# noahares/raxtax

Measured on AMD Instinct MI355X. Metric: classified queries/sec (whole node), higher is better.
Workload: dtype u32 bit-planes + f64

## Files before the change

### include/raxtax_hip.h

```cpp
#ifndef RAXTAX_HIP_H
#define RAXTAX_HIP_H

#include <stddef.h>
#include <stdint.h>

#ifdef __cplusplus
extern "C" {
#endif

#define RTX_ABI_VERSION 6
#define RTX_NUM_KMERS 65536u
#define RTX_MAX_DEPTH 32u

#define RTX_OK 0
#define RTX_ERR_INVALID (-1)
#define RTX_ERR_HIP (-2)
#define RTX_ERR_NO_DEVICE (-3)
#define RTX_ERR_OOM (-4)
#define RTX_ERR_PARSE (-5)
#define RTX_ERR_DEPTH (-6)
#define RTX_ERR_STATE (-7)
#define RTX_ERR_TOO_LONG (-8)
#define RTX_ERR_SENDER (-9)
#define RTX_RETRY_CHUNK 1
// ... 89 lines not shown
#define RTX_OPT_TILE_SKIP 10
#define RTX_OPT_LOCATOR 12
#define RTX_OPT_TILE_PRUNE 13
#define RTX_OPT_FINE_BOUNDS 17
#define RTX_OPT_RECORDS 18
#define RTX_OPT_OVERLAP 19
#define RTX_OPT_MIN_SUB_BATCHES 20
#define RTX_OPT_TWO_LEVEL_BOUNDS 21
#define RTX_OPT_PRUNE_SELF_SAMPLE 22
#define RTX_OPT_RUN_AHEAD 23
#define RTX_OPT_DEVICE_TEXT 24
#define RTX_OPT_STRAND 25
#define RTX_OPT_NEAREST 26
#define RTX_NO_REF 0xFFFFFFFFu
#define RTX_OPT_DEREP 27
int rtx_index_set_option(rtx_index *index, int option, uint64_t value);

int rtx_index_self_sample(rtx_index *index, const uint8_t *seq_bytes, const uint64_t *seq_off, uint64_t n_refs, uint32_t n_sample, double *live_fraction);
int rtx_index_prune_verdict(const rtx_index *index, int *pruning, double *live_fraction);
int rtx_index_run_ahead_stats(const rtx_index *index, uint64_t *enqueued_ahead, uint64_t *abandoned);
#define RTX_DEFAULT_SEGMENT_CLASSES 1
#define RTX_DEFAULT_EXACT_HASH_MASK 2
#define RTX_DEFAULT_DEREP_HASH_MASK 3
int rtx_set_default_option(int option, uint64_t value);

typedef struct {
    uint32_t n_queries;
    uint64_t n_rows;
    const uint32_t *t;
    const uint8_t *status;
// ... 164 lines not shown
```

### raxtax_amd/_lib.py

```python
from __future__ import annotations

import ctypes as C
from pathlib import Path

import numpy as np

PKG = Path(__file__).resolve().parent
import os as _os

LIB_PATH = Path(_os.environ.get("RTX_LIB_PATH") or PKG / "libraxtax_hip.so")

RTX_MAX_DEPTH = 32
RTX_NUM_KMERS = 65536
RTX_OK = 0
RTX_ERR_INVALID, RTX_ERR_HIP, RTX_ERR_NO_DEVICE, RTX_ERR_OOM = -1, -2, -3, -4
RTX_ERR_PARSE, RTX_ERR_DEPTH, RTX_ERR_STATE, RTX_ERR_TOO_LONG = -5, -6, -7, -8
RTX_SKIP_EXACT_MATCHES = 1
RTX_RAW_CONFIDENCE = 2
RTX_TEXT_TSV = 4
RTX_Q_OK, RTX_Q_NO_KMERS, RTX_Q_ALL_KMERS = 0, 1, 2
RTX_OPT_DEREP = 27
RTX_DEFAULT_DEREP_HASH_MASK = 3
STAGES = ("kmer_extract", "hit_count", "prob_table", "taxon_prefix", "lineage_walk", "tile_bounds", "tile_prune", "exact_match", "order", "pair_union")

u8p = C.POINTER(C.c_uint8)
u16p = C.POINTER(C.c_uint16)
u32p = C.POINTER(C.c_uint32)
u64p = C.POINTER(C.c_uint64)
f64p = C.POINTER(C.c_double)
f32p = C.POINTER(C.c_float)


class NodesView(C.Structure):
    _fields_ = [("n_nodes", C.c_uint32), ("node_begin", u32p), ("node_end", u32p), ("node_first_child", u32p),
                ("node_n_children", u32p), ("node_parent", u32p), ("node_type", u8p)]

# ... 180 lines not shown
```

### raxtax_amd/api.py

```python
from __future__ import annotations

import ctypes as C
from dataclasses import dataclass
from typing import Callable, List, Optional, Sequence, Tuple

import numpy as np

from . import _lib
from ._lib import (RTX_MAX_DEPTH, RTX_RAW_CONFIDENCE, RTX_SKIP_EXACT_MATCHES, NodesView, ResultView, RtxError, check,
                   f32p, f64p, ptr, u8p, u16p, u32p, u64p)


def _flatten(seqs: Sequence[np.ndarray]) -> Tuple[np.ndarray, np.ndarray]:
    off = np.zeros(len(seqs) + 1, dtype=np.uint64)
    if len(seqs):
        off[1:] = np.cumsum([len(s) for s in seqs], dtype=np.uint64)
    flat = np.zeros(max(int(off[-1]), 1), dtype=np.uint8)
    for i, s in enumerate(seqs):
        flat[int(off[i]):int(off[i + 1])] = np.asarray(s, dtype=np.uint8)
    return flat, off


class Tree:

# ... 210 lines not shown

DEFAULT_SEGMENT_CLASSES = 1


class Index:

    nearest_on = False

    def __init__(self, tree: Tree, device: int = 0, sub_batch: int = 0, prob_mode: int = 0,
                 stage_timing: bool = False, cluster: Optional[bool] = None, segment_classes=None,
                 packed_counts: Optional[bool] = None,
                 tile_skip: Optional[bool] = None, hit_pair=None, locator: Optional[bool] = None, tile_prune: Optional[bool] = None,
                 debug_taps: bool = False, device_exact: Optional[bool] = None, fine_bounds: Optional[bool] = None,
                 records: Optional[int] = None, overlap: Optional[bool] = None, two_level: Optional[int] = None,
                 prune_self_sample: Optional[bool] = None, device_text: bool = False, strand: str = "plus",
                 nearest: bool = False, derep: bool = False):
        self._lib = _lib.load()
        self.tree = tree
        if segment_classes is None:
            segment_classes = DEFAULT_SEGMENT_CLASSES
        check(self._lib.rtx_set_default_option(1, int(segment_classes)))
        h = C.c_void_p()
        check(self._lib.rtx_index_create_from_tree(device, tree._h, C.byref(h)))
        self._h = h
        self.n_refs = self._lib.rtx_index_num_refs(self._h)
        if sub_batch:
            check(self._lib.rtx_index_set_batch(self._h, sub_batch))
        if prob_mode:
            check(self._lib.rtx_index_set_option(self._h, 2, prob_mode))
        if stage_timing:
            check(self._lib.rtx_index_set_option(self._h, 6, 1))
# ... 25 lines not shown
            check(self._lib.rtx_index_set_option(self._h, 19, int(overlap)))
        if two_level is not None:
            check(self._lib.rtx_index_set_option(self._h, 21, int(two_level)))
        if prune_self_sample is not None:
            check(self._lib.rtx_index_set_option(self._h, 22, int(prune_self_sample)))
        if strand not in ("plus", "both"):
            raise ValueError(f"strand must be 'plus' or 'both', not {strand!r}")
        self.strand = strand
        if strand == "both":
            check(self._lib.rtx_index_set_option(self._h, 25, 1))
        self.nearest_on = bool(nearest)
        if nearest:
            check(self._lib.rtx_index_set_option(self._h, 26, 1))
        if derep:
            check(self._lib.rtx_index_set_option(self._h, _lib.RTX_OPT_DEREP, 1))
        self._view = ResultView()
        self._keep = None

    @property
    def prune_verdict(self):
        on, frac = C.c_int(), C.c_double()
        check(self._lib.rtx_index_prune_verdict(self._h, C.byref(on), C.byref(frac)))
        return bool(on.value), float(frac.value)

    @property
    def run_ahead_stats(self):
        a, b = C.c_uint64(), C.c_uint64()
        check(self._lib.rtx_index_run_ahead_stats(self._h, C.byref(a), C.byref(b)))
        return int(a.value), int(b.value)

# ... 402 lines not shown
```

### raxtax_amd/csrc/rtx_api_batch.hip

```cpp
#include "rtx_index.hpp"

#ifndef RTX_B2_HEAVY_PER_ATILE
#define RTX_B2_HEAVY_PER_ATILE 4u
#endif

namespace rtxi {

int bind(rtx_index *ix) {
    if (!ix) { set_error("null index handle"); return RTX_ERR_INVALID; }
    RTX_HIP(hipSetDevice(ix->device));
    return RTX_OK;
}

int ensure_events(rtx_index *ix, size_t count) {
    while (ix->events.size() < count) {
        hipEvent_t e;
        RTX_HIP(hipEventCreate(&e));
        ix->events.push_back(e);
    }
    return RTX_OK;
}


SubBatch sub_batch_of(rtx_index *ix, uint32_t sb, bool timed) {
// ... 70 lines not shown
    kp.rstride = k.rstride;
    kp.dmask = sc.d_dmask.p;
    kp.srows = sc.d_srows.p;
    kp.nsparse = sc.d_nsparse.p;
    kp.t = sc.d_t.p;
    kp.nrows = sc.d_nrows.p;
    kp.hq = r.d_hq.p;
    kp.t_all = r.d_t_all.p;
    kp.nrows_all = r.d_nrows_all.p;
    kp.hist = sc.d_hist.p;
    kp.hstride = k.hstride;
    return kp;
}

static bool run_prunes(const rtx_index *ix, const rtx_index::BatchClass &k) { return k.prune && !ix->dbg_full_run; }
static bool on_records_path(const rtx_index *ix, const rtx_index::BatchClass &k, const rtx_index::Scratch &sc) { return run_prunes(ix, k) && k.rec && sc.d_rec.p != nullptr; }
static bool on_diet(const rtx_index *ix, const rtx_index::BatchClass &k, const rtx_index::Scratch &sc) { return on_records_path(ix, k, sc) && k.diet && sc.d_cnt_row.p != nullptr; }

static RecordRef record_ref(const rtx_index *ix, const rtx_index::Scratch &sc, const rtx_index::ResultSet &r) { return RecordRef{sc.d_rec_nslots.p, sc.d_rec_slots.p, sc.d_rec_cnt.p, sc.d_rec.p, ix->rec_slots(), ix->rec_seg_len, r.d_flags.p}; }
static ProbTables prob_tables(const rtx_index *ix) { return ProbTables{ix->d_tab_cmf.p, ix->d_tab_ratio.p, ix->d_tab_off.p, ix->d_tab_moff.p, ix->d_tab_ilo.p, ix->d_tab_sat.p, ix->tab_tmax}; }

int enqueue_kmer(rtx_index *ix, const SubBatch &b, hipStream_t s) {
    KmerParams kp = kmer_params(ix, b);
    kp.mode = run_prunes(ix, *b.cls) && ix->seg_blocks ? 1u : 0u;
    if (b.timed_all) RTX_HIP(hipEventRecord(stage_event(ix, b, RTX_STAGE_KMER_EXTRACT, 0), s));
    launch_kmer_extract(s, kp, b.nq);
    if (b.timed_all) RTX_HIP(hipEventRecord(stage_event(ix, b, RTX_STAGE_KMER_EXTRACT, 1), s));
    return RTX_OK;
}

static HitParams hit_params(rtx_index *ix, const SubBatch &b, uint32_t flags) {
    rtx_index::Scratch &sc = ix->sc[b.set];
    rtx_index::ResultSet &r = ix->res();
    const rtx_index::BatchClass &k = *b.cls;
    HitParams hp{};
    hp.bitmap = ix->d_bitmap.p;
    hp.stride_bytes = ix->stride_bytes;
    hp.n_rows1 = ix->n_rows + 1;
    hp.n_refs = ix->n_refs;
    hp.ref_base = ix->ref_lo;
    hp.rows = sc.d_rows.p;
// ... 132 lines not shown
    fp.live_words = LiveLayout{ix->ntiles}.words();
    fp.prune_thr = sc.d_prune_thr.p;
    fp.fine_n_refs = ix->n_refs;
    fp.fine_ref_ntiles = ix->ntiles;
    fp.fine_stats = ix->d_prune_stats.p + 2 * kPruneStatCopies * 8;
    return fp;
}

int enqueue_hit(rtx_index *ix, const SubBatch &b, uint32_t flags, hipStream_t s, int part, hipStream_t s_mid) {
    rtx_index::Scratch &sc = ix->sc[b.set];
    rtx_index::ResultSet &r = ix->res();
    const rtx_index::BatchClass &k = *b.cls;
    ix->last_set = b.set;
    HitParams hp = hit_params(ix, b, flags);
    const bool prune = run_prunes(ix, k);
    if (k.pair && part != 2) {
        if (b.timed_all) RTX_HIP(hipEventRecord(stage_event(ix, b, RTX_STAGE_PAIR_UNION, 0), s));
        launch_pair_union(s, sc.d_rows.p, sc.d_nrows.p, k.rstride, b.nq, sc.d_urec.p, sc.d_nu.p, 2u * k.rstride);
        if (b.timed_all) RTX_HIP(hipEventRecord(stage_event(ix, b, RTX_STAGE_PAIR_UNION, 1), s));
    }
    if (b.timed && !prune) RTX_HIP(hipEventRecord(stage_event(ix, b, RTX_STAGE_HIT_COUNT, 0), s));
    if (part != 0 && !prune) { set_error("internal: a split run without tile pruning"); return RTX_ERR_STATE; }
    if (prune) {
        if (part != 2) {
            const HitParams up = bounds_params(ix, sc, hp);
            if (b.timed) RTX_HIP(hipEventRecord(stage_event(ix, b, RTX_STAGE_TILE_BOUNDS, 0), s));
            ix->two_level_used = part == 0 && ix->two_level_opt && ix->d_abitmap.p && ix->d_bbitmap.p && ix->n_refs == ix->n_total && k.planes <= kBounds2MaxPlanes;
            if (ix->two_level_used) {
                const bool heavy_ok = sc.d_heavy.p && sc.d_heavy_items.p && sc.d_heavy_items.n >= HeavyItemsLayout(b.nq, ix->u_ntiles).total();
                launch_bounds2(s, bounds2_params(ix, sc, up, heavy_ok), b.nq, k.planes, up, ix->u_ntiles, heavy_ok ? sc.d_heavy_items.p : nullptr);
            } else {
// ... 1003 lines not shown
```

### raxtax_amd/csrc/rtx_api_debug.hip

```cpp
#include "rtx_index.hpp"

extern "C" {

int rtx_batch_stage_times(rtx_index *ix, float ms[RTX_NUM_STAGES], uint32_t launches[RTX_NUM_STAGES]) {
    int rc = bind(ix);
    if (rc) return rc;
    if (!ix->synced) { set_error("rtx_batch_stage_times: batch not synchronised"); return RTX_ERR_STATE; }
    for (int s = 0; s < RTX_NUM_STAGES; s++) { ms[s] = 0.f; launches[s] = 0; }
    for (uint32_t sb = 0; sb < ix->n_sub_last; sb++) {
        const rtx_index::BatchClass &kc = ix->cls[ix->plan[sb].cls];
        for (int s = 0; s < RTX_NUM_STAGES; s++) {
            if (s == RTX_STAGE_EXACT_MATCH) {
                if (sb != 0 || !ix->dev_exact_used || !ix->stage_timing) continue;
            } else if (s == RTX_STAGE_ORDER) {
                if (sb != 0 || !ix->stage_timing) continue;
            } else if (s == RTX_STAGE_PAIR_UNION) {
                if (!kc.pair || !ix->stage_timing) continue;
            } else if (s == RTX_STAGE_TILE_BOUNDS || s == RTX_STAGE_TILE_PRUNE ? !kc.prune : (s != RTX_STAGE_HIT_COUNT && !ix->stage_timing)) continue;
            float t = 0.f;
            RTX_HIP(hipEventElapsedTime(&t, ix->events[((size_t)sb * RTX_NUM_STAGES + s) * 2],
                                        ix->events[((size_t)sb * RTX_NUM_STAGES + s) * 2 + 1]));
            ms[s] += t;
            launches[s]++;
        }
    }
    return RTX_OK;
}

int rtx_batch_nearest_time(rtx_index *ix, float *ms, uint32_t *launches) {
    if (!ix || !ms || !launches) { set_error("null argument"); return RTX_ERR_INVALID; }
    int rc = bind(ix);
    if (rc) return rc;
// ... 139 lines not shown
        if (row == 0xFFFFFFFFu) { set_error("debug tap: the query holds no row of the counts buffer (records path)"); return RTX_ERR_STATE; }
        slot = row;
    }
    if (!ix->packs(k.planes)) { *out = sc.d_counts.p + (size_t)slot * ix->npad; return RTX_OK; }
    int rc = ix->d_counts_dbg.alloc(ix->npad);
    if (rc) return rc;
    launch_counts_unpack(ix->stream, counts_lo(ix, sc) + (size_t)slot * ix->npad, counts_hi(ix, k, sc) + (size_t)slot * (ix->npad >> 3), ix->npad,
                         ix->d_counts_dbg.p);
    RTX_HIP(hipStreamSynchronize(ix->stream));
    *out = ix->d_counts_dbg.p;
    return RTX_OK;
}

int rtx_debug_kmers(rtx_index *ix, uint64_t query, uint16_t *kmers, uint32_t *t) {
    uint32_t slot;
    int rc = debug_slot(ix, query, &slot);
    if (rc) return rc;
    uint32_t tt = 0;
    RTX_HIP(hipMemcpy(&tt, ix->sc[ix->last_set].d_t.p + slot, 4, hipMemcpyDeviceToHost));
    if (t) *t = tt;
    if (kmers && tt) RTX_HIP(hipMemcpy(kmers, ix->sc[ix->last_set].d_kmers.p + (size_t)slot * ix->last_cls().kstride, std::min(tt, ix->last_cls().kstride) * 2, hipMemcpyDeviceToHost));
    return RTX_OK;
}

int rtx_debug_hit_counts(rtx_index *ix, uint64_t query, uint16_t *counts) {
    uint32_t slot;
    int rc = debug_slot(ix, query, &slot);
    if (rc) return rc;
    const uint16_t *src = nullptr;
    if ((rc = debug_counts_u16(ix, slot, &src))) return rc;
    RTX_HIP(hipMemcpy(counts, src, ix->n_refs * 2, hipMemcpyDeviceToHost));
// ... 286 lines not shown
```

### raxtax_amd/csrc/rtx_api_index.hip

```cpp
#include "rtx_index.hpp"

namespace rtx {
int index_device(const rtx_index *index) { return index ? index->device : -1; }
void index_set_shared_device(rtx_index *index, bool shared) { if (index) index->shared_device = shared; }
uint32_t index_swap_min_subs(rtx_index *index, uint32_t v) { if (!index) return 0; const uint32_t old = index->min_subs; index->min_subs = v; return old; }
bool index_strand(const rtx_index *index) { return index && index->strand_opt != 0u; }
bool index_nearest(const rtx_index *index) { return index && index->nearest_opt != 0u; }
bool index_profile(const rtx_index *index, uint32_t *cutoff_hundredths, uint32_t *flags) {
    if (!index || !index->prof.on) return false;
    if (cutoff_hundredths) *cutoff_hundredths = index->prof.cutoff;
    if (flags) *flags = index->prof.flags;
    return true;
}
bool index_device_text(const rtx_index *index) { return index && index->device_text_opt != 0u; }
bool index_derep(const rtx_index *index) { return index && index->derep_opt != 0u; }
uint32_t index_swap_run_ahead(rtx_index *index, uint32_t v) {
    if (!index) return 0;
    const uint32_t old = index->run_ahead_opt;
    (void)rtx_index_set_option(index, RTX_OPT_RUN_AHEAD, v);
    return old;
}
}

namespace {
// ... 743 lines not shown
        case RTX_OPT_RUN_AHEAD:
            index->run_ahead_opt = (uint32_t)std::min<uint64_t>(value, 2u);
            if (!value && index->join_pending) {
                int rc_b = bind(index);
                if (!rc_b) rc_b = settle_join(index);
                return rc_b;
            }
            return RTX_OK;
        case RTX_OPT_DEVICE_TEXT:
            index->device_text_opt = value ? 1u : 0u;
            return RTX_OK;
        case RTX_OPT_DEREP:
            if (value > 1) break;
            index->derep_opt = (uint32_t)value;
            return RTX_OK;
        case RTX_OPT_STRAND:
            if (value > 1) break;
            if (value && index->n_refs != index->n_total) { set_error("RTX_OPT_STRAND: not on a reference-shard handle (the peak of a query is spread over the shards)"); return RTX_ERR_INVALID; }
            index->uploaded = index->ran = index->synced = false;
            index->in[0].staged = index->in[1].staged = false;
            index->ws_valid = false;
            index->strand_opt = (uint32_t)value;
            return RTX_OK;
        case RTX_OPT_NEAREST:
            if (value > 1) break;
            if (value && index->n_refs != index->n_total) { set_error("RTX_OPT_NEAREST: not on a reference-shard handle (the peak of a query is spread over the shards)"); return RTX_ERR_INVALID; }
            index->uploaded = index->ran = index->synced = false;
            index->in[0].staged = index->in[1].staged = false;
            index->ws_valid = false;
            index->nearest_opt = (uint32_t)value;
// ... 37 lines not shown
```

### raxtax_amd/csrc/rtx_emul.cpp

```cpp
#include <algorithm>
#include <cmath>
#include <cstdint>
#include <cstring>
#include <array>
#include <vector>

#include "rtx_math.hpp"

using namespace rtx;

extern "C" {

uint32_t emul_planes_grouped(const uint32_t *rows, uint32_t n_rows, uint32_t groups, uint32_t *out) {
    constexpr int NP = 10;
    std::vector<std::array<uint32_t, NP>> part(groups);
    for (auto &p : part) p.fill(0);
    for (uint32_t u = 0; u + 8 * groups <= n_rows; u += 8 * groups)
        for (uint32_t g = 0; g < groups; g++) {
            const uint32_t *r = rows + u + 8 * g;
            uint32_t pl[NP];
            for (int p = 0; p < NP; p++) pl[p] = part[g][p];
            planes_ripple<NP, 3>(pl, planes_tree8<NP>(pl, r[0], r[1], r[2], r[3], r[4], r[5], r[6], r[7]));
            for (int p = 0; p < NP; p++) part[g][p] = pl[p];
        }
// ... 583 lines not shown
        const ProfileStep st = profile_step(src, q, one[q], cutoff);
        totals[0]++;
        totals[st.kind == kProfClassified ? 1 : (st.kind == kProfUnclassified ? 2 : 3)]++;
        if (st.kind != kProfClassified) continue;
        uint32_t node = st.node;
        for (uint32_t d = st.L; d-- > 0u;) {
            if (node >= n_nodes) break;
            clade[node]++;
            conf_sum[node] += st.at(d);
            if (d + 1u == st.L) direct[node]++;
            node = parent[node];
        }
    }
}

}
```

### raxtax_amd/csrc/rtx_index.hpp

```cpp
#pragma once

#include <hip/hip_runtime.h>

#include <algorithm>
#include <cmath>
#include <cstdlib>
#include <cstring>
#include <thread>

#include "rtx_internal.hpp"
#include "rtx_kernels.hpp"
#include "rtx_math.hpp"

using namespace rtx;

namespace rtxi {


constexpr uint32_t kEmptyRow = 0xFFFFFFFFu;
constexpr uint32_t kLnFactLen = 98320;

#define RTX_HIP(call)                                                                          \
    do {                                                                                       \
        hipError_t e_ = (call);                                                                \
// ... 134 lines not shown
    std::vector<uint32_t> h_em_goff, h_em_gids;
    bool dev_exact_used = false;
    struct HostExact {
        std::vector<uint32_t> grp;
        std::vector<uint64_t> off;
        std::vector<uint32_t> ids;
        bool csr_valid = false, valid = false;
    } host_exact[2];
    uint64_t n_q = 0;
    bool uploaded = false, ran = false, synced = false;
    uint32_t last_flags = 0;
    uint32_t cluster = 1;
    uint32_t packed_opt = 1;
    uint32_t tile_skip = 1;
    uint32_t pair_opt = 1;
    uint32_t prune_opt = 1;
    uint32_t self_sample_opt = 1;
    bool prune_pays = true;
    double self_live = -1.0;
    bool pruning() const { return prune_opt != 0u && (prune_pays || self_sample_opt == 0u); }
    bool dbg_full = false;
    bool dbg_full_run = false;
    DevBuf<uint32_t> d_ubitmap;
    uint32_t u_stride_bytes = 0, u_ntiles = 0;
    uint64_t u_nblocks = 0;
    DevBuf<uint32_t> d_fbitmap;
    uint32_t f_stride_bytes = 0, f_ntiles = 0;
    uint64_t f_nblocks = 0;
    uint32_t fine_opt = 1;
    DevBuf<uint32_t> d_abitmap;
// ... 54 lines not shown
    uint64_t sum_query_bytes = 0;
    uint32_t sub_batch_req = 0;
    uint32_t min_subs = 4;
    uint64_t ws_key[14] = {0};
    bool ws_valid = false;
    struct BatchClass {
        uint64_t pos0 = 0, n = 0, max_len = 0;
        uint32_t tmax = 0, kstride = 0, rstride = 0, hstride = 0, sub_batch = 0, sb0 = 0, n_sub = 0;
        int planes = 10;
        bool use_tables = false, pair = false, prune = false, rec = false, huge = false, will_prune = false;
        bool side = false;
        bool diet = false;
        uint32_t cnt_rows = 0;
    } cls[5];
    uint32_t n_cls = 0;
    uint64_t key_lim[4] = {~0ull, ~0ull, ~0ull, ~0ull};
    struct SubPlan { uint64_t q0; uint32_t nq, cls; };
    std::vector<SubPlan> plan;
    uint32_t n_sub_total() const { return (uint32_t)plan.size(); }
    uint32_t sub_batch_max = 0;
    bool any_prune = false;
    DevBuf<double> d_prob_scratch;
    struct Scratch {
        DevBuf<uint16_t> d_kmers, d_counts, d_tilemax;
        DevBuf<uint32_t> d_rows, d_t, d_nrows, d_hist, d_order, d_srows, d_nsparse;
        DevBuf<unsigned long long> d_dmask;
        DevBuf<double> d_table_z, d_prefix;
        DevBuf<uint2> d_urec;
        DevBuf<uint32_t> d_nu;
        DevBuf<uint32_t> d_live, d_best_key;
// ... 305 lines not shown
```

### raxtax_amd/csrc/rtx_kernels.hip

```cpp
#include <hip/hip_runtime.h>

#include "rtx_kernels.hpp"
#include "rtx_math.hpp"
#include "rtx_wave.hpp"
#include "rtx_hit_common.hpp"
#include "rtx_walk.hpp"

namespace rtx {

static constexpr uint32_t kEmptyRow = 0xFFFFFFFFu;

__global__ __launch_bounds__(256) void bitmap_build_kernel(const uint64_t *__restrict__ off,
                                                           const uint32_t *__restrict__ post,
                                                           const uint32_t *__restrict__ row_of,
                                                           uint32_t *__restrict__ bitmap, uint32_t stride_words, uint32_t n_rows1,
                                                           uint32_t ref_lo, uint32_t ref_hi, uint32_t shift) {
    const uint32_t k = blockIdx.x;
    const uint32_t row = row_of[k];
    if (row == kEmptyRow) return;
    const uint64_t b = off[k], e = off[k + 1];
    for (uint64_t i = b + threadIdx.x; i < e; i += blockDim.x) {
        const uint32_t g = post[i];
        if (g < ref_lo || g >= ref_hi) continue;
        uint32_t word, bit;
// ... 357 lines not shown
        if (lane < nt) {
            p.nsparse[(size_t)q * nt + lane] = cs;
            nseg += cd;
        }
    }
#pragma unroll
    for (int d = 32; d >= 1; d >>= 1) { hq += __shfl_xor(hq, d, 64); nseg += __shfl_xor(nseg, d, 64); }
    if (lane == 0) {
        if (mode != 2u) {
            p.t[q] = t > 65535u ? 0u : t;
            p.nrows[q] = nrows;
            p.hq[gq] = hq;
            p.t_all[gq] = t;
        }
        p.nrows_all[gq] = nseg;
    }
}


#ifndef RTX_HIT_NB
#define RTX_HIT_NB 2
#endif

template <int NP, bool kPacked, bool kGlobalHist = false>
#if RTX_HIT_NB > 2
__global__ __launch_bounds__(64, (RTX_HIT_NB == 3 ? 3 : 2)) void hit_count_kernel(HitParams p) {
#else
__global__ __launch_bounds__(64, (NP <= 10 ? 4 : 2)) void hit_count_kernel(HitParams p) {
#endif
    extern __shared__ uint32_t hist_lds[];
// ... 590 lines not shown
void launch_row_popcount(hipStream_t s, const uint32_t *row_of, const uint32_t *bitmap, uint32_t stride_words, uint32_t n_rows1,
                         uint32_t *list_len) {
    hipLaunchKernelGGL(row_popcount_kernel, dim3(RTX_NUM_KMERS), dim3(256), 0, s, row_of, bitmap, stride_words, n_rows1, list_len);
}
__global__ __launch_bounds__(256) void row_len_pack_kernel(const uint32_t *__restrict__ row_of, const uint32_t *__restrict__ list_len, uint2 *__restrict__ out) {
    const uint32_t k = blockIdx.x * 256u + threadIdx.x;
    out[k] = make_uint2(row_of[k], list_len[k]);
}
void launch_row_len_pack(hipStream_t s, const uint32_t *row_of, const uint32_t *list_len, uint2 *out) {
    hipLaunchKernelGGL(row_len_pack_kernel, dim3(RTX_NUM_KMERS / 256), dim3(256), 0, s, row_of, list_len, out);
}
void launch_kmer_extract(hipStream_t s, const KmerParams &p, uint32_t nq) {
    if (p.mode == 2u) hipLaunchKernelGGL(kmer_extract_kernel<true>, dim3(nq), dim3(64), 0, s, p);
    else hipLaunchKernelGGL(kmer_extract_kernel<false>, dim3(nq), dim3(64), 0, s, p);
}
constexpr uint32_t kHitLdsHistMax = 12288;
void launch_hit_count(hipStream_t s, const HitParams &p_in, uint32_t nq, uint32_t ntiles, int planes) {
    HitParams p = p_in;
    const bool ghist = p.hstride > kHitLdsHistMax;
    const uint32_t first = std::max<uint32_t>(ghist ? 0u : (p.hstride + 3u) & ~3u, kHitListCap + (RTX_HIT_NB > 2 ? 192u : 64u));
    p.lds_cnt8_off = first;
    const size_t lds = (size_t)first * sizeof(uint32_t) + 4096;
    if (ghist) hipLaunchKernelGGL((hit_count_kernel<16, false, true>), dim3(nq, ntiles), dim3(64), lds, s, p);
    else if (planes <= 10 && p.counts_lo) hipLaunchKernelGGL((hit_count_kernel<10, true>), dim3(nq, ntiles), dim3(64), lds, s, p);
    else if (planes <= 10) hipLaunchKernelGGL((hit_count_kernel<10, false>), dim3(nq, ntiles), dim3(64), lds, s, p);
    else if (planes <= 12) hipLaunchKernelGGL((hit_count_kernel<12, false>), dim3(nq, ntiles), dim3(64), lds, s, p);
    else hipLaunchKernelGGL((hit_count_kernel<16, false>), dim3(nq, ntiles), dim3(64), lds, s, p);
}
size_t prob_table_lds_bytes(uint32_t tmax) {
    const size_t n1max = tmax / 2 + 1;
// ... 44 lines not shown
```

### raxtax_amd/csrc/rtx_kernels.hpp

```cpp
#pragma once

#include <hip/hip_runtime.h>

#include <cstdint>

#include "raxtax_hip.h"
#include "rtx_math.hpp"

namespace rtx {

#ifndef RTX_NODE_TYPES_DEFINED
#define RTX_NODE_TYPES_DEFINED
enum NodeType : uint8_t { kInner = 0, kTaxon = 1, kSequence = 2 };
#endif

constexpr uint32_t kWalkMaxRows = 208;
constexpr uint32_t kSegSlotEntries = 16, kSegSparseMax = 16, kSegMaxSparseRows = 255;
constexpr uint32_t kSegPad = 8192;
__host__ __device__ inline uint32_t seg_pad(uint32_t i) { return kSegPad + ((i & 63u) << 2); }
constexpr uint32_t kKmerFewLive = 8;
constexpr uint32_t kHitListCap = 1024;

struct DevRow {
    uint32_t node;
// ... 144 lines not shown
    uint32_t *rows;
    uint32_t rstride;
    unsigned long long *dmask;
    uint32_t *srows;
    uint32_t *nsparse;
    uint32_t *t;
    uint32_t *nrows;
    unsigned long long *hq;
    uint32_t *t_all;
    uint32_t *nrows_all;
    uint32_t *hist;
    uint32_t hstride;
    uint32_t mode;
    const uint32_t *live;
    uint32_t live_words;
};

constexpr uint32_t kRecMaxSlots = 16;
struct RecordRef {
    uint16_t *nslots;
    uint16_t *slots;
    uint32_t *cnt;
    uint32_t *rec;
    uint32_t stride;
    uint32_t seg_len;
    uint32_t *flags_out;
};

struct HitParams {
    const uint32_t *bitmap;
// ... 243 lines not shown
    WalkParams walk;
    unsigned long long *prefix_stats;
    unsigned long long *stats;
};
void launch_records_tail(hipStream_t s, const TailParams &p, uint32_t nq);

void launch_bitmap_build(hipStream_t s, const uint64_t *off, const uint32_t *post, const uint32_t *row_of,
                         uint32_t *bitmap, uint32_t stride_words, uint32_t n_rows1, uint32_t ref_lo, uint32_t ref_hi, uint32_t shift = 0);
void launch_ref_kmer_mark(hipStream_t s, const uint8_t *bases, const uint64_t *off, uint64_t n_refs, uint32_t *present);
void launch_ref_bitmap_set(hipStream_t s, const uint8_t *bases, const uint64_t *off, uint64_t n_refs,
                           const uint32_t *row_of, uint32_t *bitmap, uint32_t stride_words, uint32_t n_rows1, uint32_t shift = 0);
void launch_row_len_pack(hipStream_t s, const uint32_t *row_of, const uint32_t *list_len, uint2 *out);
void launch_row_popcount(hipStream_t s, const uint32_t *row_of, const uint32_t *bitmap, uint32_t stride_words, uint32_t n_rows1,
                         uint32_t *list_len);
void launch_kmer_extract(hipStream_t s, const KmerParams &p, uint32_t nq);
void launch_hit_count(hipStream_t s, const HitParams &p, uint32_t nq, uint32_t ntiles, int planes);
void launch_pair_union(hipStream_t s, const uint32_t *rows, const uint32_t *nrows, uint32_t rstride, uint32_t nq, uint2 *urec,
                       uint32_t *nu, uint32_t ustride);
void launch_hit_count_pair(hipStream_t s, const HitParams &p, uint32_t nq, uint32_t ntiles, int planes);
void launch_live_items(hipStream_t s, const uint32_t *live, uint32_t live_words, const uint32_t *pair_live, uint32_t nq, uint32_t ntiles, uint32_t *off,
                       uint32_t *items, uint32_t *n_items);
void launch_hit_count_pair_bounds(hipStream_t s, const HitParams &p, uint32_t nq, uint32_t u_ntiles, int planes);
void launch_hit_count_pair_bounds_items(hipStream_t s, const HitParams &p, uint32_t nq, uint32_t u_ntiles, int planes);
void launch_fine_bounds(hipStream_t s, const HitParams &p, uint32_t nq, uint32_t ntiles, uint32_t f_ntiles, uint32_t *pair_live, uint32_t *cnt,
                        uint32_t *items, uint32_t *n_items, int planes);
size_t prob_table_lds_bytes(uint32_t tmax);
void launch_prob_table(hipStream_t s, const ProbParams &p, uint32_t nq);
size_t prob_lookup_lds_bytes(uint32_t tmax);
void launch_prob_tables_build(hipStream_t s, const ProbTables &tb, const double *lf, const double *inv);
void launch_prob_order(hipStream_t s, const uint32_t *t, uint32_t nq, uint32_t *order);
// ... 25 lines not shown
```

### raxtax_amd/csrc/rtx_math.hpp

```cpp
#pragma once

#include <cmath>
#include <cstdint>

#if defined(__HIPCC__)
#define RTX_HD __host__ __device__ __forceinline__
#else
#define RTX_HD inline
#endif

namespace rtx {


RTX_HD uint32_t tile_lanes(uint32_t stride_bytes, uint32_t tile) {
    const uint32_t rem = stride_bytes - tile * 1024u;
    return rem >= 1024u ? 64u : rem >> 4;
}
RTX_HD size_t bitmap_word(uint32_t row, uint32_t word, uint32_t n_rows1) {
    return ((size_t)(word >> 8) * n_rows1 + row) * 256u + (word & 255u);
}
RTX_HD void ref_slot(uint32_t r, uint32_t stride_bytes, uint32_t &word, uint32_t &bit) {
    const uint32_t tile = r >> 13, rl = r & 8191u;
    const uint32_t L = tile_lanes(stride_bytes, tile);
    const uint32_t c = rl >> 3, l = c % L, g = c / L;
// ... 14 lines not shown
        packed_count_pos(base + j, byte, hw, hs);
        byte -= base;
        hw -= base >> 3;
        const uint32_t c = ((lo[byte >> 2] >> ((byte & 3u) * 8u)) & 0xFFu) | (((hi2 >> (hw * 16u + hs)) & 3u) << 8);
        if (c == peak && base + j < in_tile) m |= 1u << j;
    }
    return m;
}
RTX_HD uint32_t nearest_match8(const uint32_t (&w)[4], uint32_t peak, uint32_t base, uint32_t in_tile) {
    uint32_t m = 0;
    for (uint32_t j = 0; j < 8u; j++) {
        const uint32_t c = (w[j >> 1] >> ((j & 1u) * 16u)) & 0xFFFFu;
        if (c == peak && base + j < in_tile) m |= 1u << j;
    }
    return m;
}

RTX_HD uint64_t em_mix_word(uint64_t w, uint64_t j) {
    uint64_t v = w + 0x9E3779B97F4A7C15ull * (j + 1u);
    v ^= v >> 32;
    v *= 0xD6E8FEB86659FD93ull;
    v ^= v >> 29;
    v *= 0xFF51AFD7ED558CCDull;
    v ^= v >> 32;
    return v;
}
RTX_HD uint64_t em_finish(uint64_t sum, uint64_t len) {
    uint64_t h = sum ^ (len * 0xC2B2AE3D27D4EB4Full);
    h ^= h >> 33;
    h *= 0xC4CEB9FE1A85EC53ull;
// ... 597 lines not shown
```

Before: 13.05 million.

## Fuse k-mer extraction and pair union into one per-pair front kernel

Adds a front_pair kernel that extracts k-mer sets for two queries at once into LDS bitmaps, merges them, and writes the per-query kmer lists, row lists and the pair-union records in one pass. It replaces the separate kmer_extract and pair_union launches on pruned pair batches with small tmax, and is on by default. This removes one launch and the global-memory round trip of row lists between the stages. The cost is a 128-thread block with heavy LDS use and several block barriers, which may lower occupancy, and it writes the histogram zeroing itself.

```diff
diff --git a/include/raxtax_hip.h b/include/raxtax_hip.h
--- a/include/raxtax_hip.h
+++ b/include/raxtax_hip.h
@@ -127,6 +127,7 @@
 #define RTX_OPT_NEAREST 26
 #define RTX_NO_REF 0xFFFFFFFFu
 #define RTX_OPT_DEREP 27
+#define RTX_OPT_FRONT_PAIR 28
 int rtx_index_set_option(rtx_index *index, int option, uint64_t value);
 
 int rtx_index_self_sample(rtx_index *index, const uint8_t *seq_bytes, const uint64_t *seq_off, uint64_t n_refs, uint32_t n_sample, double *live_fraction);
diff --git a/raxtax_amd/_lib.py b/raxtax_amd/_lib.py
--- a/raxtax_amd/_lib.py
+++ b/raxtax_amd/_lib.py
@@ -20,6 +20,7 @@
 RTX_TEXT_TSV = 4
 RTX_Q_OK, RTX_Q_NO_KMERS, RTX_Q_ALL_KMERS = 0, 1, 2
 RTX_OPT_DEREP = 27
+RTX_OPT_FRONT_PAIR = 28
 RTX_DEFAULT_DEREP_HASH_MASK = 3
 STAGES = ("kmer_extract", "hit_count", "prob_table", "taxon_prefix", "lineage_walk", "tile_bounds", "tile_prune", "exact_match", "order", "pair_union")
 
diff --git a/raxtax_amd/api.py b/raxtax_amd/api.py
--- a/raxtax_amd/api.py
+++ b/raxtax_amd/api.py
@@ -248,7 +248,7 @@
                  debug_taps: bool = False, device_exact: Optional[bool] = None, fine_bounds: Optional[bool] = None,
                  records: Optional[int] = None, overlap: Optional[bool] = None, two_level: Optional[int] = None,
                  prune_self_sample: Optional[bool] = None, device_text: bool = False, strand: str = "plus",
-                 nearest: bool = False, derep: bool = False):
+                 nearest: bool = False, derep: bool = False, front_pair: Optional[bool] = None):
         self._lib = _lib.load()
         self.tree = tree
         if segment_classes is None:
@@ -304,6 +304,8 @@
             check(self._lib.rtx_index_set_option(self._h, 26, 1))
         if derep:
             check(self._lib.rtx_index_set_option(self._h, _lib.RTX_OPT_DEREP, 1))
+        if front_pair is not None:
+            check(self._lib.rtx_index_set_option(self._h, _lib.RTX_OPT_FRONT_PAIR, int(front_pair)))
         self._view = ResultView()
         self._keep = None
 
diff --git a/raxtax_amd/csrc/rtx_api_batch.hip b/raxtax_amd/csrc/rtx_api_batch.hip
--- a/raxtax_amd/csrc/rtx_api_batch.hip
+++ b/raxtax_amd/csrc/rtx_api_batch.hip
@@ -108,6 +108,7 @@
 }
 
 static bool run_prunes(const rtx_index *ix, const rtx_index::BatchClass &k) { return k.prune && !ix->dbg_full_run; }
+static bool front_fuses(const rtx_index *ix, const rtx_index::BatchClass &k) { return run_prunes(ix, k) && ix->front_fused(k); }
 static bool on_records_path(const rtx_index *ix, const rtx_index::BatchClass &k, const rtx_index::Scratch &sc) { return run_prunes(ix, k) && k.rec && sc.d_rec.p != nullptr; }
 static bool on_diet(const rtx_index *ix, const rtx_index::BatchClass &k, const rtx_index::Scratch &sc) { return on_records_path(ix, k, sc) && k.diet && sc.d_cnt_row.p != nullptr; }
 
@@ -118,7 +119,16 @@
     KmerParams kp = kmer_params(ix, b);
     kp.mode = run_prunes(ix, *b.cls) && ix->seg_blocks ? 1u : 0u;
     if (b.timed_all) RTX_HIP(hipEventRecord(stage_event(ix, b, RTX_STAGE_KMER_EXTRACT, 0), s));
-    launch_kmer_extract(s, kp, b.nq);
+    if (front_fuses(ix, *b.cls)) {
+        rtx_index::Scratch &sc = ix->sc[b.set];
+        kp.pair_urec = sc.d_urec.p;
+        kp.pair_nu = sc.d_nu.p;
+        kp.pair_ustride = 2u * b.cls->rstride;
+        kp.nq = b.nq;
+        launch_front_pair(s, kp, b.nq);
+    } else {
+        launch_kmer_extract(s, kp, b.nq);
+    }
     if (b.timed_all) RTX_HIP(hipEventRecord(stage_event(ix, b, RTX_STAGE_KMER_EXTRACT, 1), s));
     return RTX_OK;
 }
@@ -281,7 +291,7 @@
     ix->last_set = b.set;
     HitParams hp = hit_params(ix, b, flags);
     const bool prune = run_prunes(ix, k);
-    if (k.pair && part != 2) {
+    if (k.pair && part != 2 && !front_fuses(ix, k)) {
         if (b.timed_all) RTX_HIP(hipEventRecord(stage_event(ix, b, RTX_STAGE_PAIR_UNION, 0), s));
         launch_pair_union(s, sc.d_rows.p, sc.d_nrows.p, k.rstride, b.nq, sc.d_urec.p, sc.d_nu.p, 2u * k.rstride);
         if (b.timed_all) RTX_HIP(hipEventRecord(stage_event(ix, b, RTX_STAGE_PAIR_UNION, 1), s));
diff --git a/raxtax_amd/csrc/rtx_api_debug.hip b/raxtax_amd/csrc/rtx_api_debug.hip
--- a/raxtax_amd/csrc/rtx_api_debug.hip
+++ b/raxtax_amd/csrc/rtx_api_debug.hip
@@ -15,7 +15,7 @@
             } else if (s == RTX_STAGE_ORDER) {
                 if (sb != 0 || !ix->stage_timing) continue;
             } else if (s == RTX_STAGE_PAIR_UNION) {
-                if (!kc.pair || !ix->stage_timing) continue;
+                if (!kc.pair || !ix->stage_timing || ix->front_fused(kc)) continue;
             } else if (s == RTX_STAGE_TILE_BOUNDS || s == RTX_STAGE_TILE_PRUNE ? !kc.prune : (s != RTX_STAGE_HIT_COUNT && !ix->stage_timing)) continue;
             float t = 0.f;
             RTX_HIP(hipEventElapsedTime(&t, ix->events[((size_t)sb * RTX_NUM_STAGES + s) * 2],
@@ -185,7 +185,7 @@
 
 int rtx_debug_kmers(rtx_index *ix, uint64_t query, uint16_t *kmers, uint32_t *t) {
     uint32_t slot;
-    int rc = debug_slot(ix, query, &slot);
+    int rc = debug_slot_as_run(ix, query, &slot);
     if (rc) return rc;
     uint32_t tt = 0;
     RTX_HIP(hipMemcpy(&tt, ix->sc[ix->last_set].d_t.p + slot, 4, hipMemcpyDeviceToHost));
diff --git a/raxtax_amd/csrc/rtx_api_index.hip b/raxtax_amd/csrc/rtx_api_index.hip
--- a/raxtax_amd/csrc/rtx_api_index.hip
+++ b/raxtax_amd/csrc/rtx_api_index.hip
@@ -781,6 +781,11 @@
             if (value > 1) break;
             index->derep_opt = (uint32_t)value;
             return RTX_OK;
+        case RTX_OPT_FRONT_PAIR:
+            if (value > 1) break;
+            index->uploaded = index->ran = index->synced = false;
+            index->front_pair_opt = (uint32_t)value;
+            return RTX_OK;
         case RTX_OPT_STRAND:
             if (value > 1) break;
             if (value && index->n_refs != index->n_total) { set_error("RTX_OPT_STRAND: not on a reference-shard handle (the peak of a query is spread over the shards)"); return RTX_ERR_INVALID; }
diff --git a/raxtax_amd/csrc/rtx_emul.cpp b/raxtax_amd/csrc/rtx_emul.cpp
--- a/raxtax_amd/csrc/rtx_emul.cpp
+++ b/raxtax_amd/csrc/rtx_emul.cpp
@@ -621,4 +621,17 @@
     }
 }
 
-}
+void emul_front_pair(const uint16_t *la, uint32_t n_a, const uint16_t *lb, uint32_t n_b, const uint64_t *present, const uint32_t *row_of, uint16_t *ka,
+                     uint16_t *kb, uint32_t *ra, uint32_t *rb, uint32_t *ux, uint32_t *uy, uint32_t *n) {
+    std::vector<uint64_t> sa(1024, 0), sb(1024, 0), a(1024), b(1024);
+    for (uint32_t i = 0; i < n_a; i++) sa[front_set_slot(la[i] >> 6)] |= 1ull << (la[i] & 63u);
+    for (uint32_t i = 0; i < n_b; i++) sb[front_set_slot(lb[i] >> 6)] |= 1ull << (lb[i] & 63u);
+    for (uint32_t t = 0; t < kFrontThreads; t++)
+        for (uint32_t j = 0; j < kFrontWordsPerThread; j++) {
+            a[t * kFrontWordsPerThread + j] = sa[j * kFrontThreads + t];
+            b[t * kFrontWordsPerThread + j] = sb[j * kFrontThreads + t];
+        }
+    front_pair_readout(a.data(), b.data(), present, row_of, ka, kb, ra, rb, ux, uy, n);
+}
+
+}
diff --git a/raxtax_amd/csrc/rtx_index.hpp b/raxtax_amd/csrc/rtx_index.hpp
--- a/raxtax_amd/csrc/rtx_index.hpp
+++ b/raxtax_amd/csrc/rtx_index.hpp
@@ -172,6 +172,7 @@
     uint32_t packed_opt = 1;
     uint32_t tile_skip = 1;
     uint32_t pair_opt = 1;
+    uint32_t front_pair_opt = 1;
     uint32_t prune_opt = 1;
     uint32_t self_sample_opt = 1;
     bool prune_pays = true;
@@ -256,6 +257,7 @@
         uint32_t cnt_rows = 0;
     } cls[5];
     uint32_t n_cls = 0;
+    bool front_fused(const BatchClass &k) const { return front_pair_opt != 0u && k.pair && k.prune && seg_blocks != 0u && k.tmax <= 2047u; }
     uint64_t key_lim[4] = {~0ull, ~0ull, ~0ull, ~0ull};
     struct SubPlan { uint64_t q0; uint32_t nq, cls; };
     std::vector<SubPlan> plan;
diff --git a/raxtax_amd/csrc/rtx_kernels.hip b/raxtax_amd/csrc/rtx_kernels.hip
--- a/raxtax_amd/csrc/rtx_kernels.hip
+++ b/raxtax_amd/csrc/rtx_kernels.hip
@@ -395,6 +395,170 @@
             p.t_all[gq] = t;
         }
         p.nrows_all[gq] = nseg;
+    }
+}
+
+__global__ __launch_bounds__(kFrontThreads) void front_pair_kernel(KmerParams p) {
+    __shared__ __attribute__((aligned(16))) uint32_t lds[kFrontListCap];
+    __shared__ uint32_t x1[2][2];
+    __shared__ uint32_t x2[2][2][8];
+    __shared__ unsigned long long x3[2][2];
+    const uint32_t pair = blockIdx.x, tid = threadIdx.x, lane = tid & 63u, wave = tid >> 6;
+    const uint32_t qa = pair * 2u, q = qa + wave;
+    const bool has_q = q < p.nq;
+    const unsigned long long lt_mask = (1ull << lane) - 1ull;
+    uint32_t *bm = lds + wave * 2048u;
+    for (uint32_t i = lane; i < 512u; i += 64) reinterpret_cast<uint4 *>(bm)[i] = make_uint4(0, 0, 0, 0);
+    if (has_q) {
+        uint32_t *h = p.hist + (size_t)q * p.hstride;
+        for (uint32_t i = lane; i < p.hstride; i += 64) h[i] = 0;
+    }
+    __syncthreads();
+    if (has_q) {
+        const uint64_t qin = p.perm[p.q0 + q];
+        const uint64_t b0 = p.base_off[qin];
+        const uint64_t len = p.base_off[qin + 1] - b0;
+        const uint8_t *seq = p.bases + b0;
+        if (len >= 8) {
+            const uint64_t nwin = len - 7;
+            const uint64_t wpl = (nwin + 63) / 64;
+            const uint64_t w0 = (uint64_t)lane * wpl;
+            const uint64_t w1 = w0 + wpl < nwin ? w0 + wpl : nwin;
+            for (uint64_t i = w0; i < w1; i += 16) {
+                unsigned long long v[3];
+                __builtin_memcpy(v, seq + i, 24);
+                const uint32_t nw = w1 - i < 16 ? (uint32_t)(w1 - i) : 16u;
+                uint32_t k = 0, run = 0;
+#pragma unroll
+                for (int b = 0; b < 23; b++) {
+                    const uint32_t c = (uint32_t)(v[b >> 3] >> ((b & 7) * 8)) & 0xFFu;
+                    const bool ok = c == 1u || c == 2u || c == 4u || c == 8u;
+                    k = ((k << 2) | (((uint32_t)__ffs((int)c) - 1u) & 3u)) & 0xFFFFu;
+                    run = ok ? run + 1u : 0u;
+                    if (b >= 7 && (uint32_t)(b - 7) < nw && run >= 8u) atomicOr(&bm[front_set_slot(k >> 6) * 2u + ((k >> 5) & 1u)], 1u << (k & 31u));
+                }
+            }
+        }
+    }
+    __syncthreads();
+
+    unsigned long long a[kFrontWordsPerThread], b[kFrontWordsPerThread];
+    uint32_t cu = 0, cab = 0;
+    {
+        const unsigned long long *sa = reinterpret_cast<const unsigned long long *>(lds), *sb = sa + 1024;
+#pragma unroll
+        for (uint32_t j = 0; j < kFrontWordsPerThread; j++) { a[j] = sa[j * kFrontThreads + tid]; b[j] = sb[j * kFrontThreads + tid]; }
+#pragma unroll
+        for (uint32_t j = 0; j < kFrontWordsPerThread; j++) {
+            cu += (uint32_t)__popcll(a[j] | b[j]);
+            cab += (uint32_t)__popcll(a[j]) + ((uint32_t)__popcll(b[j]) << 16);
+        }
+    }
+    const uint32_t incl_u = wave_incl_scan_u32(cu), incl_ab = wave_incl_scan_u32(cab);
+    if (lane == 63u) { x1[wave][0] = incl_u; x1[wave][1] = incl_ab; }
+    __syncthreads();
+    const uint32_t o_u = x1[wave ^ 1u][0], o_ab = x1[wave ^ 1u][1];
+    const uint32_t tot_u = (uint32_t)__builtin_amdgcn_readlane((int)incl_u, 63) + o_u, tot_ab = (uint32_t)__builtin_amdgcn_readlane((int)incl_ab, 63) + o_ab;
+    const uint32_t nu_all = tot_u < kFrontListCap ? tot_u : kFrontListCap;
+    const uint32_t t = wave ? tot_ab >> 16 : tot_ab & 0xFFFFu;
+    {
+        uint32_t pos = incl_u - cu + (wave ? o_u : 0u);
+#pragma unroll
+        for (uint32_t j = 0; j < kFrontWordsPerThread; j++) {
+            unsigned long long u = a[j] | b[j];
+            const uint32_t kbase = (tid * kFrontWordsPerThread + j) * 64u;
+            while (u) {
+                const uint32_t bit = (uint32_t)__builtin_ctzll(u);
+                u &= u - 1;
+                if (pos < kFrontListCap) lds[pos] = front_entry(kbase + bit, (a[j] >> bit) & 1ull, (b[j] >> bit) & 1ull);
+                pos++;
+            }
+        }
+    }
+    __syncthreads();
+
+    uint16_t *kout_a = p.kmers + (size_t)qa * p.kstride, *kout_b = kout_a + p.kstride;
+    uint32_t *rout_a = p.rows + (size_t)qa * p.rstride, *rout_b = rout_a + p.rstride;
+    uint2 *uout = p.pair_urec + (size_t)pair * p.pair_ustride;
+    uint32_t b_a = 0, b_b = 0, b_pa = 0, b_pb = 0, b_pu = 0;
+    unsigned long long hqa = 0, hqb = 0;
+    uint32_t par = 0;
+    for (uint32_t r0 = 0; r0 < nu_all; r0 += 1024u, par ^= 1u) {
+        const uint32_t n_r = nu_all - r0 < 1024u ? nu_all - r0 : 1024u, half = ((n_r + 127u) >> 7) << 6;
+        const uint32_t s0 = r0 + (wave ? half : 0u), s1 = r0 + (wave || half > n_r ? n_r : half);
+        uint32_t ent[8];
+        uint2 rl[8];
+#pragma unroll
+        for (int u = 0; u < 8; u++) {
+            const uint32_t i = s0 + (uint32_t)u * 64u + lane;
+            ent[u] = i < s1 ? lds[i] : 0u;
+        }
+#pragma unroll
+        for (int u = 0; u < 8; u++) {
+            rl[u] = make_uint2(kEmptyRow, 0u);
+            if (ent[u]) rl[u] = p.row_len[ent[u] & 0xFFFFu];
+        }
+        uint32_t c_a = 0, c_b = 0, c_pa = 0, c_pb = 0, c_pu = 0;
+#pragma unroll
+        for (int u = 0; u < 8; u++) {
+            const bool in_a = (ent[u] >> 16) & 1u, in_b = (ent[u] >> 17) & 1u, pres = rl[u].x != kEmptyRow;
+            c_a += (uint32_t)__popcll(__ballot(in_a));
+            c_b += (uint32_t)__popcll(__ballot(in_b));
+            c_pa += (uint32_t)__popcll(__ballot(in_a && pres));
+            c_pb += (uint32_t)__popcll(__ballot(in_b && pres));
+            c_pu += (uint32_t)__popcll(__ballot(pres));
+            hqa += in_a ? rl[u].y : 0u;
+            hqb += in_b ? rl[u].y : 0u;
+        }
+        if (lane == 0) { x2[par][wave][0] = c_a; x2[par][wave][1] = c_b; x2[par][wave][2] = c_pa; x2[par][wave][3] = c_pb; x2[par][wave][4] = c_pu; }
+        __syncthreads();
+        const uint32_t o_a = x2[par][wave ^ 1u][0], o_b = x2[par][wave ^ 1u][1], o_pa = x2[par][wave ^ 1u][2], o_pb = x2[par][wave ^ 1u][3], o_pu = x2[par][wave ^ 1u][4];
+        uint32_t p_a = b_a + (wave ? o_a : 0u), p_b = b_b + (wave ? o_b : 0u), p_pa = b_pa + (wave ? o_pa : 0u), p_pb = b_pb + (wave ? o_pb : 0u),
+                 p_pu = b_pu + (wave ? o_pu : 0u);
+#pragma unroll
+        for (int u = 0; u < 8; u++) {
+            if (s0 + (uint32_t)u * 64u >= s1) break;
+            const bool in_a = (ent[u] >> 16) & 1u, in_b = (ent[u] >> 17) & 1u, pres = rl[u].x != kEmptyRow;
+            const uint32_t k = ent[u] & 0xFFFFu;
+            const unsigned long long m_a = __ballot(in_a), m_b = __ballot(in_b), m_pa = __ballot(in_a && pres), m_pb = __ballot(in_b && pres), m_pu = __ballot(pres);
+            const uint32_t at_a = p_a + (uint32_t)__popcll(m_a & lt_mask), at_b = p_b + (uint32_t)__popcll(m_b & lt_mask);
+            const uint32_t at_pa = p_pa + (uint32_t)__popcll(m_pa & lt_mask), at_pb = p_pb + (uint32_t)__popcll(m_pb & lt_mask),
+                           at_pu = p_pu + (uint32_t)__popcll(m_pu & lt_mask);
+            if (in_a && at_a < p.kstride) kout_a[at_a] = (uint16_t)k;
+            if (in_b && at_b < p.kstride) kout_b[at_b] = (uint16_t)k;
+            if (in_a && pres && at_pa < p.rstride) rout_a[at_pa] = rl[u].x;
+            if (in_b && pres && at_pb < p.rstride) rout_b[at_pb] = rl[u].x;
+            if (pres && at_pu < p.pair_ustride) {
+                uint32_t x, y;
+                front_urec(rl[u].x, in_a, in_b, at_pa, at_pb, x, y);
+                uout[at_pu] = make_uint2(x, y);
+            }
+            p_a += (uint32_t)__popcll(m_a);
+            p_b += (uint32_t)__popcll(m_b);
+            p_pa += (uint32_t)__popcll(m_pa);
+            p_pb += (uint32_t)__popcll(m_pb);
+            p_pu += (uint32_t)__popcll(m_pu);
+        }
+        b_a += c_a + o_a;
+        b_b += c_b + o_b;
+        b_pa += c_pa + o_pa;
+        b_pb += c_pb + o_pb;
+        b_pu += c_pu + o_pu;
+    }
+#pragma unroll
+    for (int d = 32; d >= 1; d >>= 1) { hqa += __shfl_xor(hqa, d, 64); hqb += __shfl_xor(hqb, d, 64); }
+    if (lane == 0) { x3[wave][0] = hqa; x3[wave][1] = hqb; }
+    __syncthreads();
+    if (tid == 0) p.pair_nu[pair] = b_pu;
+    if (!has_q) return;
+    const uint32_t nrows = wave ? b_pb : b_pa;
+    uint32_t *rout = wave ? rout_b : rout_a;
+    for (uint32_t i = nrows + lane; i < ((nrows + 63u) & ~63u) && i < p.rstride; i += 64) rout[i] = p.zero_row;
+    if (lane == 0) {
+        p.t[q] = t;
+        p.nrows[q] = nrows;
+        p.hq[p.q0 + q] = x3[0][wave] + x3[1][wave];
+        p.t_all[p.q0 + q] = t;
     }
 }
 
@@ -1015,6 +1179,9 @@
     if (p.mode == 2u) hipLaunchKernelGGL(kmer_extract_kernel<true>, dim3(nq), dim3(64), 0, s, p);
     else hipLaunchKernelGGL(kmer_extract_kernel<false>, dim3(nq), dim3(64), 0, s, p);
 }
+void launch_front_pair(hipStream_t s, const KmerParams &p, uint32_t nq) {
+    hipLaunchKernelGGL(front_pair_kernel, dim3((nq + 1u) / 2u), dim3(kFrontThreads), 0, s, p);
+}
 constexpr uint32_t kHitLdsHistMax = 12288;
 void launch_hit_count(hipStream_t s, const HitParams &p_in, uint32_t nq, uint32_t ntiles, int planes) {
     HitParams p = p_in;
diff --git a/raxtax_amd/csrc/rtx_kernels.hpp b/raxtax_amd/csrc/rtx_kernels.hpp
--- a/raxtax_amd/csrc/rtx_kernels.hpp
+++ b/raxtax_amd/csrc/rtx_kernels.hpp
@@ -182,6 +182,10 @@
     uint32_t mode;
     const uint32_t *live;
     uint32_t live_words;
+    uint2 *pair_urec;
+    uint32_t *pair_nu;
+    uint32_t pair_ustride;
+    uint32_t nq;
 };
 
 constexpr uint32_t kRecMaxSlots = 16;
@@ -455,6 +459,7 @@
 void launch_row_popcount(hipStream_t s, const uint32_t *row_of, const uint32_t *bitmap, uint32_t stride_words, uint32_t n_rows1,
                          uint32_t *list_len);
 void launch_kmer_extract(hipStream_t s, const KmerParams &p, uint32_t nq);
+void launch_front_pair(hipStream_t s, const KmerParams &p, uint32_t nq);
 void launch_hit_count(hipStream_t s, const HitParams &p, uint32_t nq, uint32_t ntiles, int planes);
 void launch_pair_union(hipStream_t s, const uint32_t *rows, const uint32_t *nrows, uint32_t rstride, uint32_t nq, uint2 *urec,
                        uint32_t *nu, uint32_t ustride);
diff --git a/raxtax_amd/csrc/rtx_math.hpp b/raxtax_amd/csrc/rtx_math.hpp
--- a/raxtax_amd/csrc/rtx_math.hpp
+++ b/raxtax_amd/csrc/rtx_math.hpp
@@ -52,6 +52,36 @@
         if (c == peak && base + j < in_tile) m |= 1u << j;
     }
     return m;
+}
+
+constexpr uint32_t kFrontThreads = 128, kFrontWordsPerThread = 8, kFrontListCap = 4096;
+RTX_HD uint32_t front_set_slot(uint32_t w) { return (w & (kFrontWordsPerThread - 1u)) * kFrontThreads + (w >> 3); }
+RTX_HD uint32_t front_entry(uint32_t k, bool in_a, bool in_b) { return k | ((uint32_t)in_a << 16) | ((uint32_t)in_b << 17); }
+RTX_HD void front_urec(uint32_t row, bool in_a, bool in_b, uint32_t pos_a, uint32_t pos_b, uint32_t &x, uint32_t &y) {
+    x = row | ((uint32_t)in_a << 30) | ((uint32_t)in_b << 31);
+    y = (in_a ? pos_a : 0xFFFFu) | ((in_b ? pos_b : 0xFFFFu) << 16);
+}
+RTX_HD void front_pair_readout(const uint64_t *a, const uint64_t *b, const uint64_t *present, const uint32_t *row_of, uint16_t *ka, uint16_t *kb,
+                               uint32_t *ra, uint32_t *rb, uint32_t *ux, uint32_t *uy, uint32_t n[5]) {
+    uint32_t ta = 0, tb = 0, na = 0, nb = 0, nu = 0;
+    for (uint32_t w = 0; w < 1024u; w++) {
+        uint64_t u = a[w] | b[w];
+        while (u) {
+            const uint32_t bit = (uint32_t)__builtin_ctzll(u);
+            u &= u - 1u;
+            const uint32_t e = front_entry(w * 64u + bit, (a[w] >> bit) & 1u, (b[w] >> bit) & 1u);
+            const uint32_t k = e & 0xFFFFu;
+            const bool in_a = (e >> 16) & 1u, in_b = (e >> 17) & 1u;
+            if (in_a) ka[ta++] = (uint16_t)k;
+            if (in_b) kb[tb++] = (uint16_t)k;
+            if (!((present[w] >> bit) & 1u)) continue;
+            front_urec(row_of[k], in_a, in_b, na, nb, ux[nu], uy[nu]);
+            nu++;
+            if (in_a) ra[na++] = row_of[k];
+            if (in_b) rb[nb++] = row_of[k];
+        }
+    }
+    n[0] = ta; n[1] = tb; n[2] = na; n[3] = nb; n[4] = nu;
 }
 
 RTX_HD uint64_t em_mix_word(uint64_t w, uint64_t j) {
```

Measured after the change: 13.46 million, median of 6. +3.2%, better.
